# youliangtan/tennisbot-rl

Hardware: AMD Instinct MI355X
Metric: env steps/sec (whole node), SwingRacket-v0 @4096 envs/GPU (higher is better)
Workload: dtype f32

## Files before the change

include/tb_stepper.h:

```cpp
#ifndef TB_STEPPER_H
#define TB_STEPPER_H

#include <stddef.h>
#include <stdint.h>

#ifdef __cplusplus
extern "C" {
#endif

#define TB_ABI_VERSION 4

#define TB_OK 0
#define TB_E_INVAL (-1)
#define TB_E_NODEVICE (-2)
#define TB_E_PARAMS (-3)
#define TB_E_UNSUPPORTED (-4)
#define TB_E_TIMEOUT (-5)

#define TB_ENV_SWING 0
#define TB_ENV_TENNIS 1

#define TB_SWING_ACT_DIM 6
#define TB_SWING_OBS_DIM 6
#define TB_TENNIS_ACT_DIM 2
// ... 62 lines not shown
  float rest_racket_court, fric_racket_court, racket_ground_threshold;
  float ground_half[3];
  float net_half[3];
  float goal_radius, goal_half_len;
  int32_t n_hull;
  float hull_edges[TB_MAX_HULL][TB_HULL_REC];
} TbParams;

typedef struct TbHandle TbHandle;

typedef struct TbOptions {
  uint32_t struct_size;
  int32_t block;
  int32_t tennis_reg_rows;
  int32_t swing_reg_rows;
  int32_t ff_lanes_per_wave;
  int32_t ff_sort;
  int32_t ff_phases;
  int32_t ff_defer;
  int32_t ff_defer_margin;
  int32_t policy_slices;
  int32_t ff_seal;
  int32_t step_waves;
} TbOptions;

int tb_abi_version(void);
int tb_obs_dim(int env_kind);
int tb_act_dim(int env_kind);
int tb_state_words(int env_kind);
const char *tb_last_error(void);

int tb_create(const TbParams *params, const TbOptions *options_or_null, int env_kind, int n_envs, int device,
              uint64_t seed, uint64_t env_id_base, TbHandle **out);

int tb_destroy(TbHandle *h);

int tb_set_params(TbHandle *h, const TbParams *params, void *stream);
int tb_params_generation(TbHandle *h);
int tb_set_racket_scale(TbHandle *h, float scale, void *stream);

int tb_reset(TbHandle *h, const uint8_t *mask_dev, float *obs_dev, void *stream);

int tb_step(TbHandle *h, const float *actions_dev, float *obs_dev, float *reward_dev,
            uint8_t *done_dev, float *terminal_obs_dev, int32_t *substeps_dev, void *stream);

int tb_rollout(TbHandle *h, int n_steps, const float *actions_dev, float *obs_dev,
// ... 240 lines not shown
              const uint32_t *words_dev , int n_envs,
              const int32_t *env_idx_dev_or_null, int n_images, const TbCamera *camera, int width, int height,
              uint8_t *rgb_dev, uint8_t *id_dev_or_null, float *depth_dev_or_null);

int tb_swing_trace(TbHandle *h, const uint32_t *words_dev, const uint8_t *done_dev, int n_rows,
                   const float *actions_dev , int stride, int max_frames,
                   uint32_t *frames_dev , int32_t *n_frames_dev,
                   float *reward_dev, int32_t *substeps_dev, uint8_t *done_out_dev,
                   float *obs_dev_or_null , void *stream);

int tb_set_pipeline(TbHandle *h, int enable);
int tb_flush(TbHandle *h, void *stream);
#define TB_MAX_MARKS 64
int tb_mark_enable(TbHandle *h, int on);
int tb_mark_record(TbHandle *h, int k, void *stream);
int tb_mark_begin(TbHandle *h);
int tb_mark_host_wait(TbHandle *h, int k, int timeout_ms);
long long tb_mark_count(TbHandle *h, int k);
int tb_pipeline_sync(TbHandle *h, int host_wait);
int tb_phase(TbHandle *h);
int tb_phase_advance(TbHandle *h, int n_steps);
int tb_pipeline_form(TbHandle *h);
int tb_step_waves(TbHandle *h);
int tb_step_form(TbHandle *h);
int tb_pipeline_recover(TbHandle *h);

int tb_get_state(TbHandle *h, uint32_t *words, uint8_t *done, int on_device, void *stream);
int tb_set_state(TbHandle *h, const uint32_t *words, const uint8_t *done, int on_device, void *stream);

#define TB_N_COUNTERS 9
int tb_counters(TbHandle *h, uint64_t *out, void *stream);
int tb_counters_reset(TbHandle *h, void *stream);
int tb_sealed_substeps(TbHandle *h, uint64_t *out, void *stream);

int tb_diag_stream_copy(const uint32_t *src_dev, uint32_t *dst_dev, int n, int rows, int device, void *stream);
int tb_diag_idle(int waves, int microseconds, int device, void *stream);
int tb_diag_two_wave_gate(TbHandle *h, uint8_t *out_dev, void *stream);
int tb_diag_fail_alloc(int nth);

#ifdef __cplusplus
}
#endif
#endif
```

tennisbot_rl_amd/csrc/tb_kernels.hpp:

```cpp
#pragma once
#include <hip/hip_runtime.h>
#include <math.h>

#include "../../include/tb_stepper.h"
#include "tb_device.hpp"
using namespace tb;

namespace {

#define TB_COUNTER_SHARDS 64

struct KArgs {
  KParams P;
  uint32_t* words;
  uint8_t* done_state;
  const float4* hull;
  const float* actions;
  float* obs;
  float* reward;
  uint8_t* done_out;
  float* term_obs;
  int32_t* substeps;
  const uint8_t* mask;
  unsigned long long* counters;
// ... 166 lines not shown
template <int KIND>
TB_DEV void write_obs(float* dst, size_t row, const float* o) {
  if (KIND == TB_ENV_SWING) {
    float2* p = reinterpret_cast<float2*>(dst + row * 6);
    p[0] = make_float2(o[0], o[1]); p[1] = make_float2(o[2], o[3]); p[2] = make_float2(o[4], o[5]);
  } else {
    float4* p = reinterpret_cast<float4*>(dst + row * 12);
    p[0] = make_float4(o[0], o[1], o[2], o[3]); p[1] = make_float4(o[4], o[5], o[6], o[7]); p[2] = make_float4(o[8], o[9], o[10], o[11]);
  }
}

template <int KIND>
TB_DEV void load_actions(const float* actions, size_t row, float* a) {
  if (KIND == TB_ENV_SWING) {
    const float2* ap = reinterpret_cast<const float2*>(actions + row * 6);
    float2 a0 = ap[0], a1 = ap[1], a2 = ap[2];
    a[0] = a0.x; a[1] = a0.y; a[2] = a1.x; a[3] = a1.y; a[4] = a2.x; a[5] = a2.y;
  } else {
    float2 a0 = *reinterpret_cast<const float2*>(actions + row * 2);
    a[0] = a0.x; a[1] = a0.y;
  }
}

template <int KIND>
TB_DEV void reset_env(const KArgs& A, const float4* KP, int i, EnvRegs& e) {
  const KParams& P = A.P;
  unsigned long long id = A.env_id_base + (unsigned long long)i;
  uint32_t k0 = (uint32_t)A.seed, k1 = (uint32_t)(A.seed >> 32);
  uint32_t c0 = (uint32_t)id, c1 = (uint32_t)(id >> 32);
  uint32_t u[4], w[4];
  TB_DIAG_PHILOX(c0, c1, e.episode, 0u, k0, k1, u);
  vec3 zero = mk(0.0f, 0.0f, 0.0f);
  e.r.v = zero; e.r.w = zero; e.b.v = zero; e.b.w = zero;
  vec3 com = mk(P.racket_com[0], P.racket_com[1], P.racket_com[2]);
  uint32_t spin_block;
  if (KIND == TB_ENV_SWING) {
    float x = uniform(5.5f, 5.5f, u[0]), y = uniform(-4.0f, 8.0f, u[1]), z = 0.6f;
    quat q0; q0.x = 0.0f; q0.y = (float)0.24740395925452292; q0.z = 0.0f; q0.w = (float)0.96891242171064473;
    e.r.q = q0;
    e.r.p = mk(x, y, z) + rotate(q0, com);
    e.b.p = mk(x - 0.1f, y, z + 0.8f);
    float gx = uniform(-3.0f, -9.0f, u[2]), gy = uniform(-5.0f, 10.0f, u[3]);
    e.aux[0] = gx; e.aux[1] = gy; e.aux[2] = x; e.aux[3] = y; e.aux[4] = z;
    float dx = e.b.p.x - gx, dy = e.b.p.y - gy;
    e.aux[5] = sqrtf(FMA(dx, dx, dy * dy));
    spin_block = 1u;
  } else {
    TB_DIAG_PHILOX(c0, c1, e.episode, 1u, k0, k1, w);
    float x = uniform(7.5f, 5.0f, u[0]), y = uniform(-5.0f, 10.0f, u[1]), z = uniform(0.2f, 0.21f - 0.2f, u[2]);
    quat q0; q0.x = 0.0f; q0.y = 0.0f; q0.z = 0.0f; q0.w = 1.0f;
    e.r.q = q0;
    e.aux[3] = reinterpret_cast<const KParams*>(KP)->racket_scale;
    e.r.p = mk(x, y, z) + e.aux[3] * com;
    e.aux[0] = uniform(25.0f, 12.5f, u[3]);
    e.aux[1] = uniform(-10.0f, 20.0f, w[0]);
    e.aux[2] = 20.0f;
    e.aux[4] = 0.0f; e.aux[5] = 0.0f;
    e.b.p = mk(uniform(-12.0f, 6.0f, w[1]), uniform(-1.0f, 2.0f, w[2]), uniform(1.0f, 0.5f, w[3]));
    spin_block = 2u;
  }
  if (P.ball_spin_max != 0.0f) {
// ... 252 lines not shown
  }
  cnt[6] += (uint32_t)(HOST_COUNTS_FIRST ? ns - 1 : ns);
}

template <int KIND>
TB_DEV void restart_episode(const KArgs& A, const float4* KP, int i, EnvRegs& e, Manifold& M, float* o) {
  e.episode += 1u;
  reset_env<KIND>(A, KP, i, e);
  M.n = 0; M.deep = 0;
  make_obs<KIND>(e, o);
}

TB_DEV void load_ball_side(const uint32_t* w, const uint8_t* done_state, int n, int i, EnvRegs& e) {
  constexpr int K = TB_ENV_SWING;
  e.r.p = mk(ld<K>(w, TB_W_RP, n, i), ld<K>(w, TB_W_RP + 1, n, i), ld<K>(w, TB_W_RP + 2, n, i));
  e.r.q.x = ld<K>(w, TB_W_RQ, n, i); e.r.q.y = ld<K>(w, TB_W_RQ + 1, n, i); e.r.q.z = ld<K>(w, TB_W_RQ + 2, n, i); e.r.q.w = ld<K>(w, TB_W_RQ + 3, n, i);
  e.b.p = mk(ld<K>(w, TB_W_BP, n, i), ld<K>(w, TB_W_BP + 1, n, i), ld<K>(w, TB_W_BP + 2, n, i));
  e.b.v = mk(ld<K>(w, TB_W_BV, n, i), ld<K>(w, TB_W_BV + 1, n, i), ld<K>(w, TB_W_BV + 2, n, i));
  e.b.w = mk(ld<K>(w, TB_W_BW, n, i), ld<K>(w, TB_W_BW + 1, n, i), ld<K>(w, TB_W_BW + 2, n, i));
  e.aux[0] = ld<K>(w, 22, n, i); e.aux[1] = ld<K>(w, 23, n, i);
  e.step_count = (int)row_word<true>(w, Dims<K>::W - 2, n, i);
  e.done = done_state[i];
}
TB_DEV bool two_wave_rare(const KParams& P, const EnvRegs& e) {
  bool rare = e.done != TB_DONE_NO || e.step_count >= 25;
  const vec3 d = e.b.p - e.r.p;
  if ((P.flags & TB_F_RACKET_BALL) && racket_in_reach(P, d, 1.0f)) {
    vec3 ql;
    float qax;
    rare |= racket_slab<false>(P, rotate_inv(e.r.q, d), 1.0f, ql, qax);
  }
  rare |= !(ball_low_point(P, e.b) >= P.static_top + 1.0e-3f);
  return rare;
}
template <bool SHORT>
TB_DEV bool two_wave_step(const KArgs& A, EnvRegs& e, float* a, int i, bool live TB_DIAG_T0_ARG) {
  constexpr int K = TB_ENV_SWING;
  static_assert(TB_W_RQ == TB_W_RP + 3 && TB_W_RV == TB_W_RP + 7 && TB_W_RW == TB_W_RP + 10 && TB_W_BV == TB_W_BP + 3 && TB_W_BW == TB_W_BP + 6,
                "the racket's 13 rows and the ball's 9 are consecutive");
  const KParams& P = A.P;
  const bool racket_wave = threadIdx.x < 64;
  const int lane = (int)(threadIdx.x & 63);
  __shared__ float2 s_rp[64];
  __shared__ float s_ball_fin[64];
  __shared__ int s_rare;
  [[maybe_unused]] const int mk0 = racket_wave ? 0 : 8;
  if constexpr (!SHORT) {
    TB_DIAG_WAIT_LOADS(live);
    TB_DIAG_MARK(mk0);
    if (__any(live && (e.done != TB_DONE_NO || e.step_count >= 25))) return false;
  }
  if (racket_wave) {
    Racket r;
    [[maybe_unused]] uint32_t at[13];
    if constexpr (SHORT) {
#pragma unroll
      for (int k = 0; k < 13; ++k) at[k] = row_byte(TB_W_RP + k, A.n, i);
      if (live) {
        load_actions<K>(A.actions, (size_t)i, a);
        r.w = mk(ld_at(A.words, at[10]), ld_at(A.words, at[11]), ld_at(A.words, at[12]));
        r.q.x = ld_at(A.words, at[3]); r.q.y = ld_at(A.words, at[4]); r.q.z = ld_at(A.words, at[5]); r.q.w = ld_at(A.words, at[6]);
        r.v = mk(ld_at(A.words, at[7]), ld_at(A.words, at[8]), ld_at(A.words, at[9]));
        r.p = mk(ld_at(A.words, at[0]), ld_at(A.words, at[1]), ld_at(A.words, at[2]));
      }
      TB_DIAG_WAIT_LOADS(live);
      TB_DIAG_MARK(mk0);
    } else {
      r = e.r;
    }
    TB_DIAG_MARK(mk0 + 1);
    const vec3 F = mk(a[0] * 400.0f, a[1] * 400.0f, FMA(a[2], 400.0f, 4.0f * 9.81f));
    const vec3 T = mk(a[3] * 5.0f, a[4] * 5.0f, a[5] * 5.0f);
    const float speed_r = sqrtf(dot(r.v, r.v));
    racket_velocity(P, r, F, T, rotate_inv(r.q, r.w), speed_r);
    r.p = fma3(P.dt, r.v, r.p);
    s_rp[lane] = make_float2(r.p.x, r.p.y);
    racket_orientation(P, r);
    TB_DIAG_MARK(mk0 + 2);
    asm volatile("s_waitcnt lgkmcnt(0)\n\ts_barrier" ::: "memory");
    TB_DIAG_MARK(mk0 + 3);
    if (__builtin_amdgcn_readfirstlane(s_rare)) return false;
    uint32_t cnt[TB_N_COUNTERS] = {};
    if (live) {
      const float out[13] = {r.p.x, r.p.y, r.p.z, r.q.x, r.q.y, r.q.z, r.q.w, r.v.x, r.v.y, r.v.z, r.w.x, r.w.y, r.w.z};
#pragma unroll
      for (int k = 0; k < 13; ++k) {
        if constexpr (SHORT) st_at(A.words, at[k], out[k]);
        else st<K>(A.words, TB_W_RP + k, A.n, i, out[k]);
      }
      float a0 = r.p.x * 0.0f, a1 = r.p.y * 0.0f, a2 = r.p.z * 0.0f, a3 = r.q.x * 0.0f;
      a0 = FMA(r.q.y, 0.0f, a0); a1 = FMA(r.q.z, 0.0f, a1); a2 = FMA(r.q.w, 0.0f, a2); a3 = FMA(r.v.x, 0.0f, a3);
      a0 = FMA(r.v.y, 0.0f, a0); a1 = FMA(r.v.z, 0.0f, a1); a2 = FMA(r.w.x, 0.0f, a2); a3 = FMA(r.w.y, 0.0f, a3);
      a0 = FMA(r.w.z, 0.0f, a0);
      const float t = (a0 + a1) + (a2 + a3);
      if (!(t == t && s_ball_fin[lane] != 0.0f)) cnt[7]++;
    }
    flush_counters(A.counters, cnt);
    TB_DIAG_MARK(mk0 + 4);
  } else {
    [[maybe_unused]] uint32_t at[10];
    if constexpr (SHORT) {
#pragma unroll
      for (int k = 0; k < 9; ++k) at[k] = row_byte(TB_W_BP + k, A.n, i);
      at[9] = row_byte(Dims<K>::W - 2, A.n, i);
      if (live) {
        const uint32_t* w = A.words;
        e.r.p = mk(ld<K>(w, TB_W_RP, A.n, i), ld<K>(w, TB_W_RP + 1, A.n, i), ld<K>(w, TB_W_RP + 2, A.n, i));
        e.r.q.x = ld<K>(w, TB_W_RQ, A.n, i); e.r.q.y = ld<K>(w, TB_W_RQ + 1, A.n, i); e.r.q.z = ld<K>(w, TB_W_RQ + 2, A.n, i); e.r.q.w = ld<K>(w, TB_W_RQ + 3, A.n, i);
        e.b.p = mk(ld_at(w, at[0]), ld_at(w, at[1]), ld_at(w, at[2]));
        e.b.v = mk(ld_at(w, at[3]), ld_at(w, at[4]), ld_at(w, at[5]));
        e.b.w = mk(ld_at(w, at[6]), ld_at(w, at[7]), ld_at(w, at[8]));
        e.aux[0] = ld<K>(w, 22, A.n, i); e.aux[1] = ld<K>(w, 23, A.n, i);
        e.step_count = (int)word_at(w, at[9]);
        e.done = A.done_state[i];
      }
      TB_DIAG_WAIT_LOADS(live);
      TB_DIAG_MARK(mk0);
    }
    Ball b = e.b;
    const float speed_b = sqrtf(dot(b.v, b.v)), spin_b = sqrtf(dot(b.w, b.w));
    ball_velocity(P, b, mk(0.0f, 0.0f, 0.0f), speed_b, spin_b);
    b.p = fma3(P.dt, b.v, b.p);
    float a0 = b.p.x * 0.0f, a1 = b.p.y * 0.0f, a2 = b.p.z * 0.0f, a3 = b.v.x * 0.0f;
    a0 = FMA(b.v.y, 0.0f, a0); a1 = FMA(b.v.z, 0.0f, a1); a2 = FMA(b.w.x, 0.0f, a2); a3 = FMA(b.w.y, 0.0f, a3);
    a0 = FMA(b.w.z, 0.0f, a0);
    const float t = (a0 + a1) + (a2 + a3);
    s_ball_fin[lane] = t == t ? 1.0f : 0.0f;
    const bool rare = __any(live && two_wave_rare(P, e));
    if (lane == 0) s_rare = rare ? 1 : 0;
    TB_DIAG_MARK(mk0 + 1);
    TB_DIAG_MARK(mk0 + 2);
    asm volatile("s_waitcnt lgkmcnt(0)\n\ts_barrier" ::: "memory");
    TB_DIAG_MARK(mk0 + 3);
    if (rare) return false;
    if (live) {
      const float out[9] = {b.p.x, b.p.y, b.p.z, b.v.x, b.v.y, b.v.z, b.w.x, b.w.y, b.w.z};
#pragma unroll
      for (int k = 0; k < 9; ++k) {
        if constexpr (SHORT) st_at(A.words, at[k], out[k]);
        else st<K>(A.words, TB_W_BP + k, A.n, i, out[k]);
      }
      if constexpr (SHORT) word_to(A.words, at[9], (uint32_t)(e.step_count + 1));
      else row_store<true>(A.words, Dims<K>::W - 2, A.n, i, (uint32_t)(e.step_count + 1));
      float2* o = reinterpret_cast<float2*>(A.obs + (size_t)i * 6);
      o[0] = s_rp[lane]; o[1] = make_float2(b.p.x, b.p.y); o[2] = make_float2(e.aux[0], e.aux[1]);
      A.reward[i] = 0.0f;
      A.done_out[i] = 0;
      if (A.substeps) A.substeps[i] = 1;
    }
    TB_DIAG_MARK(mk0 + 4);
  }
  TB_DIAG_ADD_LANE0(mk0 + 5, 1);
  return true;
}

__global__ void __launch_bounds__(64) tb_diag_two_wave_gate_kernel(KArgs A, uint8_t* out) {
  const int i = blockIdx.x * 64 + threadIdx.x;
  if (i >= A.n) return;
// ... 4 lines not shown

}
#include "tb_policy.hpp"
namespace {

#ifndef TB_HINT_TENNIS_CONSTANTS
#define TB_HINT_TENNIS_CONSTANTS 1
#endif
#ifndef TB_HINT_TENNIS_OUTPUTS
#define TB_HINT_TENNIS_OUTPUTS 1
#endif
#ifndef TB_HINT_POLICY_VGPR_PARAMS
#define TB_HINT_POLICY_VGPR_PARAMS 1
#endif
constexpr bool step_rows_in_registers(int kind, bool lean, bool multi, bool rg, bool policy) { return !rg && (kind == TB_ENV_TENNIS || (lean && !multi && !policy)); }
constexpr bool step_has_two_waves(int kind, bool lean, bool multi, bool rg, bool policy) { return kind == TB_ENV_SWING && lean && !multi && !rg && !policy; }
constexpr int step_lds_words(int kind, bool lean, bool multi, bool rg, bool policy) { return lds_words(!step_rows_in_registers(kind, lean, multi, rg, policy), rg); }
struct StepKernelArgs { const uint32_t* words; const uint8_t* done; const float* actions; const float4* hull; int n, n_hull; KArgs A; };
TB_DEV const KArgs* refetched_args() {
  auto seg = (const __attribute__((address_space(4))) char*)__builtin_amdgcn_kernarg_segment_ptr();
  asm volatile("" : "+s"(seg));
  return (const KArgs*)(seg + offsetof(StepKernelArgs, A));
}
template <int KIND, bool LEAN, bool MULTI, bool RG, bool POLICY = false, bool TWO_WAVE = false, int NET = TB_NET_DEFAULT, bool SHORT = false>
__global__ void __launch_bounds__(256) tb_step_kernel(const uint32_t* __restrict__ k_words, const uint8_t* __restrict__ k_done, const float* __restrict__ k_actions,
                                                      const float4* __restrict__ k_hull, int k_n, int k_nhull, KArgs k_args) {
  const KArgs& A = k_args;
  constexpr int NA = Dims<KIND>::A, NO = Dims<KIND>::O;
  constexpr bool TABLE_IN_MEMORY = !POLICY && !MULTI && KIND == TB_ENV_TENNIS;
  static_assert(!TWO_WAVE || step_has_two_waves(KIND, LEAN, MULTI, RG, POLICY), "the two-wave form is the pipelined SwingRacket one-step kernel's");
  static_assert(!SHORT || TWO_WAVE, "the short form is a two-wave form");
  constexpr bool REGROWS = step_rows_in_registers(KIND, LEAN, MULTI, RG, POLICY);
  constexpr bool LAZYTAB = !POLICY && !MULTI && KIND == TB_ENV_SWING && LEAN && !RG;
  constexpr unsigned FORM = (RG ? SF_RG : 0u) | (REGROWS ? SF_REGROWS : 0u) | (LAZYTAB ? SF_LAZYTAB : 0u);
  __shared__ float4 s_lds_hull[TABLE_IN_MEMORY ? 1 : TB_HULL_LDS];
  __shared__ __attribute__((aligned(16))) float s_mean[POLICY ? 64 * 8 : 4];
  const int i = POLICY || TWO_WAVE ? blockIdx.x * 64 + (threadIdx.x & 63) : blockIdx.x * blockDim.x + threadIdx.x;
  constexpr bool SEP = KIND == TB_ENV_TENNIS;
  const uint32_t* __restrict__ w_words = SEP ? k_words : A.words;
  const uint8_t* __restrict__ w_done = SEP ? k_done : A.done_state;
  const float* __restrict__ w_actions = SEP ? k_actions : A.actions;
  const float4* __restrict__ w_hull = SEP ? k_hull : A.hull;
  const int w_n = SEP ? k_n : A.n, w_nhull = SEP ? k_nhull : A.P.n_hull;
  const float4* const s_hull = TABLE_IN_MEMORY ? w_hull : s_lds_hull;
  const bool live = i < w_n;
  EnvRegs e;
  TB_DIAG_NOW(t_entry);
  TB_DIAG_TRACE_ENTRY(trace_slot);
  TB_DIAG_CADENCE_ENTRY(cad_t0, cad_n);
  float a[NA];
  if (!SHORT && live && !(POLICY && threadIdx.x >= 64)) {
    if (TWO_WAVE && threadIdx.x >= 64) {
      load_ball_side(w_words, w_done, w_n, i, e);
    } else {
      load_env<KIND>(w_words, w_done, w_n, i, e);
      if (!POLICY) load_actions<KIND>(w_actions, (size_t)i, a);
    }
  }
  if constexpr (TWO_WAVE) {
    if (two_wave_step<SHORT>(A, e, a, i, live TB_DIAG_T0_PASS)) {
      TB_DIAG_TRACE_EXIT(trace_slot);
      TB_DIAG_CADENCE_EXIT(cad_t0, cad_n);
      return;
    }
    if (threadIdx.x >= 64) return;
  }
  const KArgs* late_args = &k_args;
  if constexpr (SHORT) late_args = refetched_args();
  {
  const KArgs& A = *late_args;
  const float4* __restrict__ w_hull = SEP ? k_hull : A.hull;
  const int w_nhull = SEP ? k_nhull : A.P.n_hull;
  if constexpr (SHORT) {
    if (live) load_env<KIND>(A.words, A.done_state, A.n, i, e);
  }
#if TB_HINT_TENNIS_CONSTANTS
  if constexpr (KIND == TB_ENV_TENNIS && !POLICY && !MULTI) {
    asm volatile("" :: "s"(A.P.dt), "s"(A.P.gravity), "s"(A.P.lin_damp), "s"(A.P.lin_damp_quad), "s"(A.P.racket_inv_mass), "s"(A.P.ball_inv_mass),
                 "s"(A.P.hull_bound_radius), "s"(A.P.hull_margin), "s"(A.P.ball_radius), "s"(A.P.contact_threshold), "s"(A.P.static_top), "s"(A.P.max_ang_step));
  }
#endif
#if TB_HINT_TENNIS_OUTPUTS
  if constexpr (KIND == TB_ENV_TENNIS && !POLICY && !MULTI)
// ... 469 lines not shown
```

tennisbot_rl_amd/csrc/tb_stepper.hip:

```cpp
#include <hip/hip_runtime.h>
#include <math.h>
#include <stdio.h>
#include <stdlib.h>
#include <string.h>
#include <chrono>
#include <type_traits>

#include "../../include/tb_stepper.h"
#include "tb_device.hpp"

#include "tb_kernels.hpp"
#include "tb_es.hpp"
#include "tb_learner.hpp"
#include "tb_trpo.hpp"
#include "tb_sac.hpp"
#include "tb_tqc.hpp"
#include "tb_render.hpp"
#include "tb_trace.hpp"

using namespace tb;

namespace {

thread_local char g_err[512] = "";
// ... 182 lines not shown
  void release() { drop(rec); drop(dst); drop(count); drop(ev_run); drop(ev_direct); *this = Pool{}; }
};

struct Marks {
  unsigned long long* h;
  unsigned long long snap_ff[TB_FF_SLOTS], snap_marks[TB_MAX_MARKS];
  int on;
  long long ff_before[TB_MAX_MARKS][TB_FF_SLOTS];
  int in_capture[TB_MAX_MARKS];
  int ensure() {
    if (h) return TB_OK;
    HIP_TRY(hipHostMalloc((void**)&h, sizeof(unsigned long long) * (TB_MAX_MARKS + TB_FF_SLOTS), hipHostMallocDefault));
    memset(h, 0, sizeof(unsigned long long) * (TB_MAX_MARKS + TB_FF_SLOTS));
    return TB_OK;
  }
};

}

struct TbHandle {
  int device, kind, n, block;
  TbOptions opt;
  int two_wave;
  uint64_t seed, env_id_base;
  TbParams params;
  KParams kp;
  uint32_t* d_words;
  uint8_t* d_done;
  float4* d_hull;
  float4* h_hull;
  float cull_planes[TB_N_CULL][3];
  unsigned long long* d_counters;
  uint32_t* d_mani;
  uint8_t* d_mflag;
  int params_generation;
  unsigned long long first_substeps;
  float* d_es_rew;
  int pipeline;
  int ff_phases;
  int ff_lanes;
  Phase phase;
  Slots slots;
  Pool pool;
  Marks marks;
};

// ... 200 lines not shown
    HIP_TRY(hipEventRecord(pool.ev_run, s));
    pool.idle(); pool.run_ev_valid = 1;
  }
  return TB_OK;
}

int run_pool_for_mark(TbHandle* h, hipStream_t s) {
  if (!(h->pool.episodes > h->pool.run_upto)) return TB_OK;
  const int slot = h->slots.claim();
  if (int rc = fork_side(h->slots.s[slot], s)) return rc;
  if (int rc = run_pool(h, h->slots.s[slot].side)) return rc;
  return close_side(h, slot, nullptr, nullptr, s);
}

int defer_mode(const TbHandle* h) {
  if (!h->pool.rec || h->opt.ff_defer < 0) return 0;
  if (h->opt.ff_defer > 0) return h->marks.on && h->opt.ff_defer == 1 ? 0 : h->opt.ff_defer;
  if (h->marks.on) return 0;
  if (h->n <= 16384) return 2;
  return (h->kp.flags & TB_F_RACKET_GROUND) ? 1 : 0;
}

struct Park { bool direct; int slot; };
int claim_park(TbHandle* h, bool may_park, KArgs& a, hipStream_t s, Park* p) {
  *p = Park{false, -1};
  if (!may_park) return TB_OK;
  a.defer = 1;
  Pool& pool = h->pool;
  if (pool.rec && defer_mode(h) == 2 && h->phase.valid && !a.term_obs && !a.substeps && pool.episodes < pool.cap / h->n) {
    if (pool.run_ev_valid) HIP_TRY(hipStreamWaitEvent(s, pool.ev_run, 0));
    a.ff_rec = pool.rec + (size_t)pool.episodes * h->n * pool_rec(h); a.ff_flag = nullptr;
    a.pool_dst_out = pool.dst + (size_t)pool.episodes * h->n;
    p->direct = true;
    return TB_OK;
  }
  p->slot = h->slots.claim();
  const FfSlot& f = h->slots.s[p->slot];
  if (f.busy) HIP_TRY(hipStreamWaitEvent(s, f.ev_ff, 0));
  a.ff_rec = f.rec; a.ff_flag = f.flag;
  return TB_OK;
}
int finish_park(TbHandle* h, const Park& p, KArgs a, size_t reward_step_stride, hipStream_t s) {
  if (p.direct) {
    HIP_TRY(hipEventRecord(h->pool.ev_direct, s));
    h->pool.direct_ev_valid = 1; h->pool.episodes++; h->pool.pending = 1;
    return TB_OK;
  }
  if (p.slot < 0) return TB_OK;
  a.reward += (size_t)(a.T - 1) * reward_step_stride;
  return launch_ff(h, p.slot, a, s);
}

int count_first_substeps(TbHandle* h, int T, hipStream_t s) {
  hipStreamCaptureStatus st;
  if (int rc = capture_status(s, &st)) return rc;
  if (st == hipStreamCaptureStatusNone) h->first_substeps += (unsigned long long)h->n * (unsigned long long)T;
  return TB_OK;
}

struct PolicyIO {
  const float* weights; const float* obs_in; float* actions; float* raw; float* logp; float* value;
  unsigned long long seed; int deterministic;
  int net;
  void apply(KArgs& a) const {
    a.pol_weights = weights; a.pol_obs = obs_in; a.pol_actions = actions; a.pol_raw = raw; a.pol_logp = logp;
    a.pol_value = value; a.pol_seed = seed; a.pol_deterministic = deterministic;
  }
};

enum { TB_STEP_ONE_WAVE = 0, TB_STEP_TWO_WAVE_GATE = 1, TB_STEP_TWO_WAVE_SHORT = 2 };
int step_form(const TbHandle* h, bool lean, bool multi, bool rg, bool policy) {
  if (!h->two_wave || !step_has_two_waves(h->kind, lean, multi, rg, policy)) return TB_STEP_ONE_WAVE;
  if (!h->phase.valid) return TB_STEP_TWO_WAVE_GATE;
  return h->phase.launch_ends_episode(1) ? TB_STEP_ONE_WAVE : TB_STEP_TWO_WAVE_SHORT;
}

int launch_step(TbHandle* h, int T, const float* actions, float* obs, float* reward, uint8_t* done, float* term, int32_t* substeps, hipStream_t s,
                const PolicyIO* pol = nullptr, bool lean_multi = false) {
  if (int rc = count_first_substeps(h, T, s)) return rc;
  KArgs a = base_args(h);
  if (pol) pol->apply(a);
  a.actions = actions; a.obs = obs; a.reward = reward; a.done_out = done; a.term_obs = term; a.substeps = substeps; a.T = T;
  dim3 grid((unsigned)((h->n + h->block - 1) / h->block)), block((unsigned)h->block);
  if (pol) { grid = dim3((unsigned)((h->n + 63) / 64)); block = dim3(256); }
  const bool piped = (T == 1 || lean_multi) && h->pipeline && h->kind == TB_ENV_SWING && (h->kp.flags & TB_F_AUTO_RESET);
  const bool may_park = piped && ((T == 1 && !h->phase.valid) || h->phase.launch_ends_episode(T));
  Park park;
  if (int rc = claim_park(h, may_park, a, s, &park)) return rc;
  const bool rg = extended_contacts(h->kp);
  const bool multi = T > 1, policy = pol != nullptr;
  const int form = step_form(h, piped, multi, rg, policy);
  const bool two_wave = form != TB_STEP_ONE_WAVE;
  const StepKernel kern = form == TB_STEP_TWO_WAVE_SHORT ? tb_step_kernel<TB_ENV_SWING, true, false, false, false, true, TB_NET_DEFAULT, true>
                                                         : step_kernel(h->kind, piped, multi, rg, policy, two_wave, pol ? pol->net : TB_NET_DEFAULT);
  if (!kern) return fail(TB_E_UNSUPPORTED, "no tb_step_kernel instantiation for this variant");
  if (two_wave) { grid = dim3((unsigned)((h->n + 63) / 64)); block = dim3(128); }
  const size_t lds = dyn_lds(step_lds_words(h->kind, piped, multi, rg, policy), policy ? 64u : block.x);
  (void)hipGetLastError();
  if (int rc = launch(kern, grid, block, lds, s, a.words, a.done_state, a.actions, a.hull, a.n, a.P.n_hull, a)) return rc;
  if (int rc = finish_park(h, park, a, h->n, s)) return rc;
  h->phase.advance(T);
  return TB_OK;
}

int refusal(int code, const char* who, const char* what) {
  char msg[320];
  snprintf(msg, sizeof msg, "%s%s", who, what);
  return fail(code, msg);
}
dim3 slice_groups(const TbHandle* h) { return dim3((unsigned)((h->n + TB_POLICY_SLICE - 1) / TB_POLICY_SLICE)); }
int members_refused(const char* who, const TbHandle* h, int n_members, int envs_per_member, int granule, size_t stride_floats, int min_floats, const void* base) {
  char msg[160];
  if (n_members < 1 || envs_per_member < 1 || envs_per_member % granule) {
    snprintf(msg, sizeof msg, ": n_members must be >= 1 and envs_per_member a positive multiple of the member granule (%d)", granule);
    return refusal(TB_E_INVAL, who, msg);
  }
// ... 135 lines not shown
int tb_act_dim(int k) { return k == TB_ENV_SWING ? TB_SWING_ACT_DIM : k == TB_ENV_TENNIS ? TB_TENNIS_ACT_DIM : TB_E_INVAL; }
int tb_state_words(int k) { return kind_ok(k) ? words_of(k) : TB_E_INVAL; }
const char* tb_last_error(void) { return g_err; }

int tb_create(const TbParams* params, const TbOptions* options, int env_kind, int n_envs, int device, uint64_t seed, uint64_t env_id_base, TbHandle** out) {
  if (!params || !out) return fail(TB_E_INVAL, "tb_create: null argument");
  *out = nullptr;
  if (!kind_ok(env_kind)) return fail(TB_E_INVAL, "tb_create: unknown env kind");
  if (n_envs <= 0 || n_envs > (1 << 25)) return fail(TB_E_INVAL, "tb_create: n_envs must be in [1, 2^25]");
  if (int rc = validate_params(params)) return rc;
  TbOptions opt;
  memset(&opt, 0, sizeof opt);
  if (options) {
    if (options->struct_size < sizeof(uint32_t) || options->struct_size > 4096) return fail(TB_E_INVAL, "tb_create: TbOptions.struct_size is not set");
    memcpy(&opt, options, options->struct_size < sizeof opt ? options->struct_size : sizeof opt);
    if (opt.block != 0 && opt.block != 64 && opt.block != 128 && opt.block != 256) return fail(TB_E_INVAL, "tb_create: TbOptions.block must be 0, 64, 128 or 256");
    if (opt.ff_lanes_per_wave < 0 || opt.ff_lanes_per_wave > 64) return fail(TB_E_INVAL, "tb_create: TbOptions.ff_lanes_per_wave must be in [0, 64]");
    if (opt.ff_phases < 0 || opt.ff_phases > 3) return fail(TB_E_INVAL, "tb_create: TbOptions.ff_phases must be in [0, 3]");
    if (opt.policy_slices != 0 && opt.policy_slices != 1 && opt.policy_slices != 3) return fail(TB_E_INVAL, "tb_create: TbOptions.policy_slices must be 0, 1 or 3");
    if (opt.ff_defer < -1 || opt.ff_defer > 2) return fail(TB_E_INVAL, "tb_create: TbOptions.ff_defer must be -1, 0, 1 or 2");
    if (opt.ff_defer_margin < 0 || opt.ff_defer_margin > 800) return fail(TB_E_INVAL, "tb_create: TbOptions.ff_defer_margin must be in [0, 800]");
    if (opt.ff_seal < -1 || opt.ff_seal > 1) return fail(TB_E_INVAL, "tb_create: TbOptions.ff_seal must be -1, 0 or 1");
    if (opt.step_waves < 0 || opt.step_waves > 2) return fail(TB_E_INVAL, "tb_create: TbOptions.step_waves must be 0, 1 or 2");
  }
  int ndev = 0;
  hipError_t e = hipGetDeviceCount(&ndev);
  if (e != hipSuccess || ndev <= 0) return fail(TB_E_NODEVICE, "tb_create: no HIP device available (this library has no CPU fallback)");
  if (device < 0 || device >= ndev) return fail(TB_E_NODEVICE, "tb_create: device index out of range");
  DeviceGuard g(device);
  if (g.err != hipSuccess) return fail((int)g.err, "hipSetDevice");

  TbHandle* h = (TbHandle*)calloc(1, sizeof(TbHandle));
  if (!h) return fail(TB_E_INVAL, "tb_create: out of host memory");
  h->device = device; h->kind = env_kind; h->n = n_envs; h->seed = seed; h->env_id_base = env_id_base;
  h->params = *params; to_kparams(params, &h->kp, &h->cull_planes[0][0]); h->block = pick_block(env_kind, n_envs, opt);
  h->opt = opt;
  h->two_wave = opt.step_waves ? opt.step_waves == 2 : n_envs <= TB_TWO_WAVE_MAX_ENVS;
  h->ff_phases = opt.ff_phases >= 1 && opt.ff_phases <= 3 ? opt.ff_phases : (n_envs >= 262144 ? 3 : 1);
  h->ff_lanes = opt.ff_lanes_per_wave;
  if (!h->ff_lanes) { h->ff_lanes = 4; while (h->ff_lanes < 64 && (long long)h->ff_lanes * 64 < n_envs) h->ff_lanes <<= 1; }
  const int nw = words_of(env_kind);
  hipError_t err;
#define CREATE_TRY(expr) if ((err = (expr)) != hipSuccess) { int rc = fail((int)err, #expr); tb_destroy(h); return rc; }
  CREATE_TRY(hipMalloc((void**)&h->d_words, sizeof(uint32_t) * (size_t)nw * n_envs));
  CREATE_TRY(hipMalloc((void**)&h->d_done, (size_t)n_envs));
  CREATE_TRY(hipMalloc((void**)&h->d_hull, sizeof(float4) * TB_HULL_LDS));
  CREATE_TRY(hipHostMalloc((void**)&h->h_hull, sizeof(float4) * TB_HULL_LDS, hipHostMallocDefault));
  CREATE_TRY(hipMalloc((void**)&h->d_counters, sizeof(unsigned long long) * kCounterWords));
  CREATE_TRY(hipMemsetAsync(h->d_counters, 0, sizeof(unsigned long long) * kCounterWords, 0));
  CREATE_TRY(hipMalloc((void**)&h->d_mani, sizeof(uint32_t) * (size_t)TB_MANI_WORDS * n_envs));
  CREATE_TRY(hipMalloc((void**)&h->d_mflag, (size_t)n_envs));
  CREATE_TRY(hipMemsetAsync(h->d_mflag, 0, (size_t)n_envs, 0));
  if (int rc = launch(tb_init_kernel, dim3((unsigned)((n_envs + 255) / 256)), dim3(256), 0, 0, h->d_words, h->d_done, n_envs, nw)) { tb_destroy(h); return rc; }
  if (int rc = upload_hull(h, 0)) { tb_destroy(h); return rc; }
  CREATE_TRY(hipStreamSynchronize(0));
#undef CREATE_TRY
  *out = h;
  return TB_OK;
}

// ... 70 lines not shown
}

int tb_phase(TbHandle* h) {
  if (!h) return fail(TB_E_INVAL, "tb_phase: null handle");
  return h->phase.valid ? h->phase.at : -1;
}

int tb_pipeline_form(TbHandle* h) {
  if (!h) return fail(TB_E_INVAL, "tb_pipeline_form: null handle");
  if (h->kind != TB_ENV_SWING || !h->pipeline) return 0;
  const int mode = defer_mode(h);
  return mode == 2 ? 3 : mode == 1 && h->ff_phases == 1 ? 2 : 1;
}

int tb_step_waves(TbHandle* h) {
  if (!h) return fail(TB_E_INVAL, "tb_step_waves: null handle");
  if (h->kind != TB_ENV_SWING || !h->pipeline) return 0;
  return h->two_wave ? 2 : 1;
}

int tb_step_form(TbHandle* h) {
  if (!h) return fail(TB_E_INVAL, "tb_step_form: null handle");
  if (h->kind != TB_ENV_SWING || !h->pipeline || !(h->kp.flags & TB_F_AUTO_RESET)) return -1;
  return step_form(h, true, false, extended_contacts(h->kp), false);
}

int tb_phase_advance(TbHandle* h, int n_steps) {
  if (!h || n_steps < 0) return fail(TB_E_INVAL, "tb_phase_advance: bad argument");
  h->phase.advance(n_steps);
  h->first_substeps += (unsigned long long)h->n * (unsigned long long)n_steps;
  return TB_OK;
}

int tb_mark_record(TbHandle* h, int k, void* stream) {
  if (!h || k < 0 || k >= TB_MAX_MARKS) return fail(TB_E_INVAL, "tb_mark_record: bad handle or mark index");
  DeviceGuard g(h->device);
  hipStream_t s = (hipStream_t)stream;
  if (!h->marks.on) return fail(TB_E_UNSUPPORTED, "tb_mark_record needs tb_mark_enable(h, 1) before the steps it covers (their fast-forwards must be counted)");
  hipStreamCaptureStatus st;
  if (int rc = capture_status(s, &st)) return rc;
  if (int rc = run_pool_for_mark(h, s)) return rc;
  if (int rc = launch(tb_mark_kernel, dim3(1), dim3(1), 0, s, h->marks.h + k)) return rc;
  h->marks.in_capture[k] = st == hipStreamCaptureStatusActive;
  for (int q = 0; q < TB_FF_SLOTS; ++q) h->marks.ff_before[k][q] = h->marks.in_capture[k] ? h->slots.s[q].in_capture : h->slots.s[q].eager;
  return TB_OK;
}

// ... 1314 lines not shown
```

tennisbot_rl_amd/params.py:

```python
import ctypes
import json
import math
import os

import numpy as np

TB_MAX_HULL = 64
TB_HULL_REC = 8

ENV_SWING = 0
ENV_TENNIS = 1
NET_DEFAULT = 0
NET_TUNED = 1
NET_MLP64 = 2
NET_NAMES = {NET_DEFAULT: "default", NET_TUNED: "tuned", NET_MLP64: "mlp64"}

F_AUTO_RESET = 0x1
F_NET = 0x2
F_RACKET_BALL = 0x4
F_RACKET_GROUND = 0x8
F_DEFAULT = F_NET | F_RACKET_BALL

DONE_NO, DONE_PENDING_FORCE, DONE_YES = 0, 1, 2

# ... 31 lines not shown
        ("rest_racket", ctypes.c_float), ("rest_court", ctypes.c_float), ("rest_goal", ctypes.c_float),
        ("fric_racket", ctypes.c_float), ("fric_court", ctypes.c_float), ("fric_goal", ctypes.c_float),
        ("roll_racket", ctypes.c_float), ("roll_court", ctypes.c_float), ("roll_goal", ctypes.c_float),
        ("rest_racket_court", ctypes.c_float), ("fric_racket_court", ctypes.c_float), ("racket_ground_threshold", ctypes.c_float),
        ("ground_half", ctypes.c_float * 3), ("net_half", ctypes.c_float * 3),
        ("goal_radius", ctypes.c_float), ("goal_half_len", ctypes.c_float),
        ("n_hull", ctypes.c_int32), ("hull_edges", (ctypes.c_float * TB_HULL_REC) * TB_MAX_HULL),
    ]

    def copy(self):
        out = TbParams()
        ctypes.memmove(ctypes.byref(out), ctypes.byref(self), ctypes.sizeof(TbParams))
        return out

    def hull_vertices(self):
        e = np.ctypeslib.as_array(self.hull_edges)[: self.n_hull]
        return e[:, :2].astype(np.float64)


class TbOptions(ctypes.Structure):
    _fields_ = [("struct_size", ctypes.c_uint32), ("block", ctypes.c_int32), ("tennis_reg_rows", ctypes.c_int32),
                ("swing_reg_rows", ctypes.c_int32), ("ff_lanes_per_wave", ctypes.c_int32), ("ff_sort", ctypes.c_int32),
                ("ff_phases", ctypes.c_int32), ("ff_defer", ctypes.c_int32), ("ff_defer_margin", ctypes.c_int32),
                ("policy_slices", ctypes.c_int32), ("ff_seal", ctypes.c_int32), ("step_waves", ctypes.c_int32)]


def make_options(block=0, tennis_reg_rows=None, swing_reg_rows=None, ff_lanes_per_wave=0, ff_sort=None, ff_phases=0, policy_slices=0, ff_defer=None, ff_defer_margin=0,
                 ff_seal=None, step_waves=0):
    def tri(x):
        return 0 if x is None else (1 if x else -1)
    o = TbOptions()
    o.struct_size = ctypes.sizeof(TbOptions)
    o.block, o.tennis_reg_rows, o.swing_reg_rows = int(block), tri(tennis_reg_rows), tri(swing_reg_rows)
    o.ff_lanes_per_wave, o.ff_sort, o.ff_phases = int(ff_lanes_per_wave), tri(ff_sort), int(ff_phases)
    o.policy_slices, o.ff_defer_margin = int(policy_slices), int(ff_defer_margin)
    o.ff_seal = tri(ff_seal)
    o.step_waves = int(step_waves)
    o.ff_defer = 2 if ff_defer == "all" else tri(ff_defer)
    return o


def load_scene(path=_ASSETS):
    with open(path) as f:
        return json.load(f)


def hull_edge_table(hull_yz_link, com_yz, scale):
    v = (np.asarray(hull_yz_link, dtype=np.float64) - np.asarray(com_yz, dtype=np.float64)) * float(scale)
    v = v.astype(np.float32).astype(np.float64)
    e = np.roll(v, -1, axis=0) - v
    l2 = (e ** 2).sum(1)
    rec = np.zeros((len(v), TB_HULL_REC), dtype=np.float64)
    rec[:, 0:2] = v
    rec[:, 2:4] = e
    rec[:, 4] = 1.0 / l2
    rec[:, 5] = 1.0 / np.sqrt(l2)
    return rec.astype(np.float32)


def bullet_shape_inertia(scene=None, hull_margin=0.001):
# ... 84 lines not shown
```

Before: 944.8 million.

## Add two-wave episode-end step form that parks episodes and respawns in-kernel

Adds a third two-wave step kernel variant for the launch that ends an episode. Before, that launch fell back to the one-wave kernel. The new form writes the final racket and ball state into the fast-forward pool record and computes the fresh spawn state in the same kernel, then stores the reset state, observations, reward and done flags. It is enabled by default when two-wave stepping is on and direct parking is possible. In exchange it adds a vmcnt wait at the barrier, more shared memory, and more complex correctness conditions, such as the step_count == 25 check and the pool-region requirement.

```diff
diff --git a/include/tb_stepper.h b/include/tb_stepper.h
--- a/include/tb_stepper.h
+++ b/include/tb_stepper.h
@@ -108,6 +108,7 @@
   int32_t policy_slices;
   int32_t ff_seal;
   int32_t step_waves;
+  int32_t episode_end_waves;
 } TbOptions;
 
 int tb_abi_version(void);
@@ -394,6 +395,7 @@
 int tb_phase_advance(TbHandle *h, int n_steps);
 int tb_pipeline_form(TbHandle *h);
 int tb_step_waves(TbHandle *h);
+#define TB_STEP_TWO_WAVE_END 3
 int tb_step_form(TbHandle *h);
 int tb_pipeline_recover(TbHandle *h);
 
diff --git a/tennisbot_rl_amd/csrc/tb_kernels.hpp b/tennisbot_rl_amd/csrc/tb_kernels.hpp
--- a/tennisbot_rl_amd/csrc/tb_kernels.hpp
+++ b/tennisbot_rl_amd/csrc/tb_kernels.hpp
@@ -212,6 +212,10 @@
   }
 }
 
+TB_DEV quat swing_spawn_quat() {
+  quat q0; q0.x = 0.0f; q0.y = (float)0.24740395925452292; q0.z = 0.0f; q0.w = (float)0.96891242171064473;
+  return q0;
+}
 template <int KIND>
 TB_DEV void reset_env(const KArgs& A, const float4* KP, int i, EnvRegs& e) {
   const KParams& P = A.P;
@@ -226,7 +230,7 @@
   uint32_t spin_block;
   if (KIND == TB_ENV_SWING) {
     float x = uniform(5.5f, 5.5f, u[0]), y = uniform(-4.0f, 8.0f, u[1]), z = 0.6f;
-    quat q0; q0.x = 0.0f; q0.y = (float)0.24740395925452292; q0.z = 0.0f; q0.w = (float)0.96891242171064473;
+    const quat q0 = swing_spawn_quat();
     e.r.q = q0;
     e.r.p = mk(x, y, z) + rotate(q0, com);
     e.b.p = mk(x - 0.1f, y, z + 0.8f);
@@ -525,8 +529,7 @@
   e.step_count = (int)row_word<true>(w, Dims<K>::W - 2, n, i);
   e.done = done_state[i];
 }
-TB_DEV bool two_wave_rare(const KParams& P, const EnvRegs& e) {
-  bool rare = e.done != TB_DONE_NO || e.step_count >= 25;
+TB_DEV bool two_wave_rare_geometry(const KParams& P, const EnvRegs& e, bool rare) {
   const vec3 d = e.b.p - e.r.p;
   if ((P.flags & TB_F_RACKET_BALL) && racket_in_reach(P, d, 1.0f)) {
     vec3 ql;
@@ -536,7 +539,10 @@
   rare |= !(ball_low_point(P, e.b) >= P.static_top + 1.0e-3f);
   return rare;
 }
-template <bool SHORT>
+TB_DEV bool two_wave_rare(const KParams& P, const EnvRegs& e) {
+  return two_wave_rare_geometry(P, e, e.done != TB_DONE_NO || e.step_count >= 25);
+}
+template <bool SHORT, bool END = false>
 TB_DEV bool two_wave_step(const KArgs& A, EnvRegs& e, float* a, int i, bool live TB_DIAG_T0_ARG) {
   constexpr int K = TB_ENV_SWING;
   static_assert(TB_W_RQ == TB_W_RP + 3 && TB_W_RV == TB_W_RP + 7 && TB_W_RW == TB_W_RP + 10 && TB_W_BV == TB_W_BP + 3 && TB_W_BW == TB_W_BP + 6,
@@ -547,6 +553,8 @@
   __shared__ float2 s_rp[64];
   __shared__ float s_ball_fin[64];
   __shared__ int s_rare;
+  static_assert(!END || SHORT, "the episode-end form loads as the short form does");
+  __shared__ float s_spawn[END ? 3 : 1][64];
   [[maybe_unused]] const int mk0 = racket_wave ? 0 : 8;
   if constexpr (!SHORT) {
     TB_DIAG_WAIT_LOADS(live);
@@ -577,14 +585,28 @@
     const float speed_r = sqrtf(dot(r.v, r.v));
     racket_velocity(P, r, F, T, rotate_inv(r.q, r.w), speed_r);
     r.p = fma3(P.dt, r.v, r.p);
-    s_rp[lane] = make_float2(r.p.x, r.p.y);
+    if constexpr (!END) s_rp[lane] = make_float2(r.p.x, r.p.y);
     racket_orientation(P, r);
     TB_DIAG_MARK(mk0 + 2);
-    asm volatile("s_waitcnt lgkmcnt(0)\n\ts_barrier" ::: "memory");
+    if constexpr (END) asm volatile("s_waitcnt vmcnt(0) lgkmcnt(0)\n\ts_barrier" ::: "memory");
+    else asm volatile("s_waitcnt lgkmcnt(0)\n\ts_barrier" ::: "memory");
     TB_DIAG_MARK(mk0 + 3);
     if (__builtin_amdgcn_readfirstlane(s_rare)) return false;
     uint32_t cnt[TB_N_COUNTERS] = {};
-    if (live) {
+    if constexpr (END) {
+      if (live) {
+        float4* rec = A.ff_rec + (size_t)i * ff_rec<false>();
+        rec[0] = make_float4(r.p.x, r.p.y, r.p.z, r.q.x);
+        rec[1] = make_float4(r.q.y, r.q.z, r.q.w, r.v.x);
+        rec[2] = make_float4(r.v.y, r.v.z, r.w.x, r.w.y);
+        rec[3].x = r.w.z;
+        const quat q0 = swing_spawn_quat();
+        const float out[13] = {s_spawn[0][lane], s_spawn[1][lane], s_spawn[2][lane], q0.x, q0.y, q0.z, q0.w, 0.0f, 0.0f, 0.0f, 0.0f, 0.0f, 0.0f};
+#pragma unroll
+        for (int k = 0; k < 13; ++k) st_at(A.words, at[k], out[k]);
+        cnt[5]++;
+      }
+    } else if (live) {
       const float out[13] = {r.p.x, r.p.y, r.p.z, r.q.x, r.q.y, r.q.z, r.q.w, r.v.x, r.v.y, r.v.z, r.w.x, r.w.y, r.w.z};
 #pragma unroll
       for (int k = 0; k < 13; ++k) {
@@ -602,10 +624,16 @@
     TB_DIAG_MARK(mk0 + 4);
   } else {
     [[maybe_unused]] uint32_t at[10];
+    [[maybe_unused]] uint32_t at_reset[7];
     if constexpr (SHORT) {
 #pragma unroll
       for (int k = 0; k < 9; ++k) at[k] = row_byte(TB_W_BP + k, A.n, i);
       at[9] = row_byte(Dims<K>::W - 2, A.n, i);
+      if constexpr (END) {
+#pragma unroll
+        for (int k = 0; k < 6; ++k) at_reset[k] = row_byte(22 + k, A.n, i);
+        at_reset[6] = row_byte(Dims<K>::W - 1, A.n, i);
+      }
       if (live) {
         const uint32_t* w = A.words;
         e.r.p = mk(ld<K>(w, TB_W_RP, A.n, i), ld<K>(w, TB_W_RP + 1, A.n, i), ld<K>(w, TB_W_RP + 2, A.n, i));
@@ -613,7 +641,13 @@
         e.b.p = mk(ld_at(w, at[0]), ld_at(w, at[1]), ld_at(w, at[2]));
         e.b.v = mk(ld_at(w, at[3]), ld_at(w, at[4]), ld_at(w, at[5]));
         e.b.w = mk(ld_at(w, at[6]), ld_at(w, at[7]), ld_at(w, at[8]));
-        e.aux[0] = ld<K>(w, 22, A.n, i); e.aux[1] = ld<K>(w, 23, A.n, i);
+        if constexpr (END) {
+#pragma unroll
+          for (int k = 0; k < 6; ++k) e.aux[k] = ld_at(w, at_reset[k]);
+          e.episode = word_at(w, at_reset[6]);
+        } else {
+          e.aux[0] = ld<K>(w, 22, A.n, i); e.aux[1] = ld<K>(w, 23, A.n, i);
+        }
         e.step_count = (int)word_at(w, at[9]);
         e.done = A.done_state[i];
       }
@@ -628,15 +662,46 @@
     a0 = FMA(b.v.y, 0.0f, a0); a1 = FMA(b.v.z, 0.0f, a1); a2 = FMA(b.w.x, 0.0f, a2); a3 = FMA(b.w.y, 0.0f, a3);
     a0 = FMA(b.w.z, 0.0f, a0);
     const float t = (a0 + a1) + (a2 + a3);
-    s_ball_fin[lane] = t == t ? 1.0f : 0.0f;
-    const bool rare = __any(live && two_wave_rare(P, e));
+    if constexpr (!END) s_ball_fin[lane] = t == t ? 1.0f : 0.0f;
+    const bool rare = __any(live && (END ? two_wave_rare_geometry(P, e, e.done != TB_DONE_NO || e.step_count != 25) : two_wave_rare(P, e)));
     if (lane == 0) s_rare = rare ? 1 : 0;
+    [[maybe_unused]] EnvRegs fresh;
+    [[maybe_unused]] float fresh_obs[6];
+    if constexpr (END) {
+      Manifold none;
+      fresh.episode = e.episode;
+      restart_episode<K>(A, A.hull + TB_HULL_KP, i, fresh, none, fresh_obs);
+      s_spawn[0][lane] = fresh.r.p.x; s_spawn[1][lane] = fresh.r.p.y; s_spawn[2][lane] = fresh.r.p.z;
+    }
     TB_DIAG_MARK(mk0 + 1);
     TB_DIAG_MARK(mk0 + 2);
-    asm volatile("s_waitcnt lgkmcnt(0)\n\ts_barrier" ::: "memory");
+    if constexpr (END) asm volatile("s_waitcnt vmcnt(0) lgkmcnt(0)\n\ts_barrier" ::: "memory");
+    else asm volatile("s_waitcnt lgkmcnt(0)\n\ts_barrier" ::: "memory");
     TB_DIAG_MARK(mk0 + 3);
     if (rare) return false;
-    if (live) {
+    if constexpr (END) {
+      if (live) {
+        float4* rec = A.ff_rec + (size_t)i * ff_rec<false>();
+        rec[3].y = b.p.x;
+        *reinterpret_cast<float2*>(&rec[3].z) = make_float2(b.p.y, b.p.z);
+        rec[4] = make_float4(b.v.x, b.v.y, b.v.z, b.w.x);
+        rec[5] = make_float4(b.w.y, b.w.z, e.aux[0], e.aux[1]);
+        rec[6] = make_float4(e.aux[2], e.aux[3], e.aux[4], e.aux[5]);
+        rec[7] = make_float4(__int_as_float(e.step_count + 1), __uint_as_float(e.episode), __uint_as_float(REC_PARKED), __int_as_float(i));
+        A.pool_dst_out[i] = A.reward + i;
+        const float out[9] = {fresh.b.p.x, fresh.b.p.y, fresh.b.p.z, fresh.b.v.x, fresh.b.v.y, fresh.b.v.z, fresh.b.w.x, fresh.b.w.y, fresh.b.w.z};
+#pragma unroll
+        for (int k = 0; k < 9; ++k) st_at(A.words, at[k], out[k]);
+#pragma unroll
+        for (int k = 0; k < 6; ++k) st_at(A.words, at_reset[k], fresh.aux[k]);
+        word_to(A.words, at_reset[6], fresh.episode);
+        word_to(A.words, at[9], (uint32_t)fresh.step_count);
+        A.done_state[i] = (uint8_t)fresh.done;
+        write_obs<K>(A.obs, (size_t)i, fresh_obs);
+        A.reward[i] = 0.0f;
+        A.done_out[i] = 1;
+      }
+    } else if (live) {
       const float out[9] = {b.p.x, b.p.y, b.p.z, b.v.x, b.v.y, b.v.z, b.w.x, b.w.y, b.w.z};
 #pragma unroll
       for (int k = 0; k < 9; ++k) {
@@ -687,7 +752,7 @@
   asm volatile("" : "+s"(seg));
   return (const KArgs*)(seg + offsetof(StepKernelArgs, A));
 }
-template <int KIND, bool LEAN, bool MULTI, bool RG, bool POLICY = false, bool TWO_WAVE = false, int NET = TB_NET_DEFAULT, bool SHORT = false>
+template <int KIND, bool LEAN, bool MULTI, bool RG, bool POLICY = false, bool TWO_WAVE = false, int NET = TB_NET_DEFAULT, bool SHORT = false, bool END = false>
 __global__ void __launch_bounds__(256) tb_step_kernel(const uint32_t* __restrict__ k_words, const uint8_t* __restrict__ k_done, const float* __restrict__ k_actions,
                                                       const float4* __restrict__ k_hull, int k_n, int k_nhull, KArgs k_args) {
   const KArgs& A = k_args;
@@ -695,6 +760,7 @@
   constexpr bool TABLE_IN_MEMORY = !POLICY && !MULTI && KIND == TB_ENV_TENNIS;
   static_assert(!TWO_WAVE || step_has_two_waves(KIND, LEAN, MULTI, RG, POLICY), "the two-wave form is the pipelined SwingRacket one-step kernel's");
   static_assert(!SHORT || TWO_WAVE, "the short form is a two-wave form");
+  static_assert(!END || SHORT, "the episode-end form is a short form");
   constexpr bool REGROWS = step_rows_in_registers(KIND, LEAN, MULTI, RG, POLICY);
   constexpr bool LAZYTAB = !POLICY && !MULTI && KIND == TB_ENV_SWING && LEAN && !RG;
   constexpr unsigned FORM = (RG ? SF_RG : 0u) | (REGROWS ? SF_REGROWS : 0u) | (LAZYTAB ? SF_LAZYTAB : 0u);
@@ -723,7 +789,7 @@
     }
   }
   if constexpr (TWO_WAVE) {
-    if (two_wave_step<SHORT>(A, e, a, i, live TB_DIAG_T0_PASS)) {
+    if (two_wave_step<SHORT, END>(A, e, a, i, live TB_DIAG_T0_PASS)) {
       TB_DIAG_TRACE_EXIT(trace_slot);
       TB_DIAG_CADENCE_EXIT(cad_t0, cad_n);
       return;
diff --git a/tennisbot_rl_amd/csrc/tb_stepper.hip b/tennisbot_rl_amd/csrc/tb_stepper.hip
--- a/tennisbot_rl_amd/csrc/tb_stepper.hip
+++ b/tennisbot_rl_amd/csrc/tb_stepper.hip
@@ -228,6 +228,8 @@
   int device, kind, n, block;
   TbOptions opt;
   int two_wave;
+  int two_wave_end;
+  int late_outputs;
   uint64_t seed, env_id_base;
   TbParams params;
   KParams kp;
@@ -474,12 +476,16 @@
 }
 
 struct Park { bool direct; int slot; };
+bool parks_direct(const TbHandle* h, bool late_outputs) {
+  const Pool& pool = h->pool;
+  return pool.rec && defer_mode(h) == 2 && h->phase.valid && !late_outputs && pool.episodes < pool.cap / h->n;
+}
 int claim_park(TbHandle* h, bool may_park, KArgs& a, hipStream_t s, Park* p) {
   *p = Park{false, -1};
   if (!may_park) return TB_OK;
   a.defer = 1;
   Pool& pool = h->pool;
-  if (pool.rec && defer_mode(h) == 2 && h->phase.valid && !a.term_obs && !a.substeps && pool.episodes < pool.cap / h->n) {
+  if (parks_direct(h, a.term_obs || a.substeps)) {
     if (pool.run_ev_valid) HIP_TRY(hipStreamWaitEvent(s, pool.ev_run, 0));
     a.ff_rec = pool.rec + (size_t)pool.episodes * h->n * pool_rec(h); a.ff_flag = nullptr;
     a.pool_dst_out = pool.dst + (size_t)pool.episodes * h->n;
@@ -521,10 +527,11 @@
 };
 
 enum { TB_STEP_ONE_WAVE = 0, TB_STEP_TWO_WAVE_GATE = 1, TB_STEP_TWO_WAVE_SHORT = 2 };
-int step_form(const TbHandle* h, bool lean, bool multi, bool rg, bool policy) {
+int step_form(const TbHandle* h, bool lean, bool multi, bool rg, bool policy, bool late_outputs) {
   if (!h->two_wave || !step_has_two_waves(h->kind, lean, multi, rg, policy)) return TB_STEP_ONE_WAVE;
   if (!h->phase.valid) return TB_STEP_TWO_WAVE_GATE;
-  return h->phase.launch_ends_episode(1) ? TB_STEP_ONE_WAVE : TB_STEP_TWO_WAVE_SHORT;
+  if (!h->phase.launch_ends_episode(1)) return TB_STEP_TWO_WAVE_SHORT;
+  return h->two_wave_end && parks_direct(h, late_outputs) ? TB_STEP_TWO_WAVE_END : TB_STEP_ONE_WAVE;
 }
 
 int launch_step(TbHandle* h, int T, const float* actions, float* obs, float* reward, uint8_t* done, float* term, int32_t* substeps, hipStream_t s,
@@ -537,13 +544,16 @@
   if (pol) { grid = dim3((unsigned)((h->n + 63) / 64)); block = dim3(256); }
   const bool piped = (T == 1 || lean_multi) && h->pipeline && h->kind == TB_ENV_SWING && (h->kp.flags & TB_F_AUTO_RESET);
   const bool may_park = piped && ((T == 1 && !h->phase.valid) || h->phase.launch_ends_episode(T));
+  const bool rg = extended_contacts(h->kp);
+  const bool multi = T > 1, policy = pol != nullptr;
+  const int form = step_form(h, piped, multi, rg, policy, term || substeps);
+  if (T == 1 && !pol) h->late_outputs = term || substeps;
   Park park;
   if (int rc = claim_park(h, may_park, a, s, &park)) return rc;
-  const bool rg = extended_contacts(h->kp);
-  const bool multi = T > 1, policy = pol != nullptr;
-  const int form = step_form(h, piped, multi, rg, policy);
+  if (form == TB_STEP_TWO_WAVE_END && !(park.direct && a.pool_dst_out)) return fail(TB_E_UNSUPPORTED, "the episode-end step form needs a pool region");
   const bool two_wave = form != TB_STEP_ONE_WAVE;
   const StepKernel kern = form == TB_STEP_TWO_WAVE_SHORT ? tb_step_kernel<TB_ENV_SWING, true, false, false, false, true, TB_NET_DEFAULT, true>
+                          : form == TB_STEP_TWO_WAVE_END ? tb_step_kernel<TB_ENV_SWING, true, false, false, false, true, TB_NET_DEFAULT, true, true>
                                                          : step_kernel(h->kind, piped, multi, rg, policy, two_wave, pol ? pol->net : TB_NET_DEFAULT);
   if (!kern) return fail(TB_E_UNSUPPORTED, "no tb_step_kernel instantiation for this variant");
   if (two_wave) { grid = dim3((unsigned)((h->n + 63) / 64)); block = dim3(128); }
@@ -725,6 +735,7 @@
     if (opt.ff_defer_margin < 0 || opt.ff_defer_margin > 800) return fail(TB_E_INVAL, "tb_create: TbOptions.ff_defer_margin must be in [0, 800]");
     if (opt.ff_seal < -1 || opt.ff_seal > 1) return fail(TB_E_INVAL, "tb_create: TbOptions.ff_seal must be -1, 0 or 1");
     if (opt.step_waves < 0 || opt.step_waves > 2) return fail(TB_E_INVAL, "tb_create: TbOptions.step_waves must be 0, 1 or 2");
+    if (opt.episode_end_waves < 0 || opt.episode_end_waves > 2) return fail(TB_E_INVAL, "tb_create: TbOptions.episode_end_waves must be 0, 1 or 2");
   }
   int ndev = 0;
   hipError_t e = hipGetDeviceCount(&ndev);
@@ -739,6 +750,7 @@
   h->params = *params; to_kparams(params, &h->kp, &h->cull_planes[0][0]); h->block = pick_block(env_kind, n_envs, opt);
   h->opt = opt;
   h->two_wave = opt.step_waves ? opt.step_waves == 2 : n_envs <= TB_TWO_WAVE_MAX_ENVS;
+  h->two_wave_end = h->two_wave && (opt.episode_end_waves ? opt.episode_end_waves == 2 : opt.step_waves == 0);
   h->ff_phases = opt.ff_phases >= 1 && opt.ff_phases <= 3 ? opt.ff_phases : (n_envs >= 262144 ? 3 : 1);
   h->ff_lanes = opt.ff_lanes_per_wave;
   if (!h->ff_lanes) { h->ff_lanes = 4; while (h->ff_lanes < 64 && (long long)h->ff_lanes * 64 < n_envs) h->ff_lanes <<= 1; }
@@ -855,7 +867,7 @@
 int tb_step_form(TbHandle* h) {
   if (!h) return fail(TB_E_INVAL, "tb_step_form: null handle");
   if (h->kind != TB_ENV_SWING || !h->pipeline || !(h->kp.flags & TB_F_AUTO_RESET)) return -1;
-  return step_form(h, true, false, extended_contacts(h->kp), false);
+  return step_form(h, true, false, extended_contacts(h->kp), false, h->late_outputs != 0);
 }
 
 int tb_phase_advance(TbHandle* h, int n_steps) {
diff --git a/tennisbot_rl_amd/params.py b/tennisbot_rl_amd/params.py
--- a/tennisbot_rl_amd/params.py
+++ b/tennisbot_rl_amd/params.py
@@ -77,11 +77,12 @@
     _fields_ = [("struct_size", ctypes.c_uint32), ("block", ctypes.c_int32), ("tennis_reg_rows", ctypes.c_int32),
                 ("swing_reg_rows", ctypes.c_int32), ("ff_lanes_per_wave", ctypes.c_int32), ("ff_sort", ctypes.c_int32),
                 ("ff_phases", ctypes.c_int32), ("ff_defer", ctypes.c_int32), ("ff_defer_margin", ctypes.c_int32),
-                ("policy_slices", ctypes.c_int32), ("ff_seal", ctypes.c_int32), ("step_waves", ctypes.c_int32)]
+                ("policy_slices", ctypes.c_int32), ("ff_seal", ctypes.c_int32), ("step_waves", ctypes.c_int32),
+                ("episode_end_waves", ctypes.c_int32)]
 
 
 def make_options(block=0, tennis_reg_rows=None, swing_reg_rows=None, ff_lanes_per_wave=0, ff_sort=None, ff_phases=0, policy_slices=0, ff_defer=None, ff_defer_margin=0,
-                 ff_seal=None, step_waves=0):
+                 ff_seal=None, step_waves=0, episode_end_waves=0):
     def tri(x):
         return 0 if x is None else (1 if x else -1)
     o = TbOptions()
@@ -90,7 +91,7 @@
     o.ff_lanes_per_wave, o.ff_sort, o.ff_phases = int(ff_lanes_per_wave), tri(ff_sort), int(ff_phases)
     o.policy_slices, o.ff_defer_margin = int(policy_slices), int(ff_defer_margin)
     o.ff_seal = tri(ff_seal)
-    o.step_waves = int(step_waves)
+    o.step_waves, o.episode_end_waves = int(step_waves), int(episode_end_waves)
     o.ff_defer = 2 if ff_defer == "all" else tri(ff_defer)
     return o
 
```

New measurement: 972.8 million (median of 5 runs). 1.03x the previous value.
